# AnishDelft/ModelCompression

Measured on AMD Instinct MI355X. Metric: images/sec (fwd+bwd, 416x416), higher is better.
Workload: dtype fp16

## Files before the change

### modelcompression_amd/csrc/api.hip

```cpp
#include <stdarg.h>
#include <stdlib.h>
#include <string.h>

#include <string>

#include "kernels.h"

static thread_local char g_err[512] = "";

void mcamd_set_error(const char* fmt, ...) {
    va_list ap;
    va_start(ap, fmt);
    vsnprintf(g_err, sizeof(g_err), fmt, ap);
    va_end(ap);
}

int g_mcamd_env_generation = 0;
int McamdEnvSlot::get(const char* name, int dflt) {
    const int g = __atomic_load_n(&g_mcamd_env_generation, __ATOMIC_ACQUIRE);
    if (gen != g) {
        const char* s = getenv(name);
        has = s && *s ? 1 : 0;
        val = has ? atoi(s) : 0;
        __atomic_store_n(&gen, g, __ATOMIC_RELEASE);
// ... 1091 lines not shown
    if (!g || g->stem) return 0;
    const ConvRoute r = dgrad_route(g, concurrent != 0, MCAMD_EPI_RAW_F16);
    return mcamd_igemm_sums_ok(r) ? r.rows : 0;
}

extern "C" int mcamd_conv_dgrad_sums(const mcamd_conv_geom* g, const void* dy, int32_t dy_ld, int32_t dy_choff,
                                     const void* wp_dgrad, const mcamd_conv_epilogue* epi, const mcamd_dgrad_sums* sums,
                                     void* stream) {
    if (mcamd_recording()) {
        MCAMD_REQUIRE(g && epi, "conv_dgrad: null geometry / epilogue");
        const mcamd_conv_geom g_ = *g;
        const mcamd_conv_epilogue e_ = *epi;
        if (!sums) return mcamd_rec_push(stream, [=](void* s) { return mcamd_conv_dgrad_sums(&g_, dy, dy_ld, dy_choff, wp_dgrad, &e_, nullptr, s); });
        const mcamd_dgrad_sums s_ = *sums;
        return mcamd_rec_push(stream, [=](void* s) { return mcamd_conv_dgrad_sums(&g_, dy, dy_ld, dy_choff, wp_dgrad, &e_, &s_, s); });
    }
    if (check_geom(g, "conv_dgrad")) return MCAMD_EINVAL;
    MCAMD_REQUIRE(g->x_wrap == 0 && g->x_f8 == 0, "conv_dgrad: x_wrap / x_f8 are forward-only fields");
    MCAMD_REQUIRE(!g->stem, "conv_dgrad: the stem layer has no input gradient");
    MCAMD_REQUIRE(dy && wp_dgrad, "conv_dgrad: null input");
    int cout_p = cout_p_of(g);
    MCAMD_REQUIRE(dy_ld % 8 == 0 && dy_choff % 8 == 0 && dy_choff + cout_p <= dy_ld,
                  "conv_dgrad: dy slice [%d, %d) does not fit dy_ld %d", dy_choff, dy_choff + cout_p, dy_ld);
    IgemmArgs a;
    fill_operand(a, g, dy, wp_dgrad, dy_ld, dy_choff, g->cin, cout_p, 0);
    MCAMD_REQUIRE(epi && epi->mode != MCAMD_EPI_PAD_F16 && !epi->stats && epi->dst_mode == 0 && !epi->y2,
                  "conv_dgrad: epilogue must be mode 0 (no stats) or 1");
    a.concurrent = epi->concurrent != 0;
    const ConvRoute r = dgrad_route(g, a.concurrent, epi->mode);
    if (fill_epilogue(a, epi, g->cin, "conv_dgrad", r.rows)) return MCAMD_EINVAL;
    if (sums && sums->slab) {
        const mcamd_dgrad_sums* s = sums;
        MCAMD_REQUIRE(epi->mode == MCAMD_EPI_RAW_F16, "conv_dgrad: producer sums go with epilogue mode 0");
        MCAMD_REQUIRE(mcamd_igemm_sums_ok(r) && s->rows == r.rows,
                      "conv_dgrad: sums.rows must be mcamd_conv_dgrad_sums_rows() = %d (got %d; 0: this launch cannot take sums)",
                      mcamd_igemm_sums_ok(r) ? r.rows : 0, s->rows);
        MCAMD_REQUIRE(s->act && s->scale && s->shift && s->mean && s->invstd, "conv_dgrad: sums: null argument");
        MCAMD_REQUIRE(s->C > 0 && s->C % 8 == 0 && s->ch_lo >= 0 && s->ch_lo % 8 == 0 && s->ch_lo + s->C <= g->cin,
                      "conv_dgrad: sums: producer columns [%d, %d) must be whole groups of 8 inside the %d channels of G",
                      s->ch_lo, s->ch_lo + s->C, g->cin);
        MCAMD_REQUIRE(s->ld >= s->C, "conv_dgrad: sums.ld (%d) must be >= C (%d)", s->ld, s->C);
        MCAMD_REQUIRE(s->act_ld % 8 == 0 && s->act_choff % 8 == 0 && s->act_choff >= 0 && s->act_choff + s->C <= s->act_ld &&
                          (s->act_pad == 0 || s->act_pad == 1),
                      "conv_dgrad: sums: activation slice [%d, %d) does not fit act_ld %d", s->act_choff, s->act_choff + s->C, s->act_ld);
        MCAMD_REQUIRE(!s->y || (s->y_ld % 4 == 0 && s->y_choff % 4 == 0 && s->y_choff >= 0 && s->y_choff + s->C <= s->y_ld),
                      "conv_dgrad: sums: fp32 y slice [%d, %d) does not fit y_ld %d", s->y_choff, s->y_choff + s->C, s->y_ld);
        MCAMD_REQUIRE(s->slope > 0.f, "conv_dgrad: sums need an invertible activation (slope > 0)");
        a.bsum.slab = s->slab, a.bsum.ld = s->ld;
        a.bsum.act = (const half_t*)s->act, a.bsum.act_ld = s->act_ld, a.bsum.act_choff = s->act_choff, a.bsum.act_pw = s->act_pad ? 1 : 2;
        a.bsum.scale = s->scale, a.bsum.shift = s->shift, a.bsum.mean = s->mean, a.bsum.invstd = s->invstd;
        a.bsum.y = s->y, a.bsum.y_ld = s->y_ld, a.bsum.y_choff = s->y_choff;
        a.bsum.ch_lo = s->ch_lo, a.bsum.C = s->C;
        a.bsum.slope = s->slope;
    }
    return launch_route(a, r, g, (hipStream_t)stream);
}

extern "C" int mcamd_conv_dgrad(const mcamd_conv_geom* g, const void* dy, int32_t dy_ld, int32_t dy_choff,
                                const void* wp_dgrad, const mcamd_conv_epilogue* epi, void* stream) {
    return mcamd_conv_dgrad_sums(g, dy, dy_ld, dy_choff, wp_dgrad, epi, nullptr, stream);
}

static WgradPlan wgrad_plan_for(const mcamd_conv_geom* g) {
    if (mcamd_wgrad_stem_ok(g->stem, g->cout, g->W, (long long)g->B * g->H * g->W))
        return mcamd_wgrad_stem_plan((long long)g->B * g->H * g->W);
    if (mcamd_wgrad_win_ok(g->ksize, g->stem, g->cout, cin_tap_of(g), g->W, (long long)g->B * g->H * g->W))
        return mcamd_wgrad_win_plan((long long)g->B * g->H * g->W, g->cout);
    if (mcamd_wgrad_use9(g->ksize, g->stem, g->cout, cin_tap_of(g), g->W))
        return mcamd_wgrad_plan9(padded_pixels(g), g->cout, cin_tap_of(g), g->W, g->W + pw_of(g), g->B);
    return mcamd_wgrad_plan((long long)g->B * g->H * g->W, g->cout, cin_tap_of(g), ntaps_of(g));
}

extern "C" size_t mcamd_conv_wgrad_workspace_bytes(const mcamd_conv_geom* g) {
    if (!g) return 0;
    return wgrad_plan_for(g).bytes;
}

extern "C" int mcamd_conv_wgrad_plan_info(const mcamd_conv_geom* g, int32_t has_cmap, int32_t out[MCAMD_WGRAD_PLAN_INFO_N]) {
    if (check_geom(g, "conv_wgrad_plan_info")) return MCAMD_EINVAL;
    MCAMD_REQUIRE(out, "conv_wgrad_plan_info: null output");
    MCAMD_REQUIRE(!(g->stem && has_cmap), "conv_wgrad_plan_info: the stem layer takes no input-channel map");
    const WgradPlan p = wgrad_plan_for(g);
    const WgradFinish f = mcamd_wgrad_finish_pick(p.nsplit, g->stem, g->cin, g->ksize, has_cmap != 0);
    const int tiles = p.n_otiles * p.n_tapgroups * p.n_ctiles;
    out[0] = p.nine == 2 ? MCAMD_WGRAD_NINE_WIDE : p.nine ? MCAMD_WGRAD_NINE : p.stemw == 1 ? MCAMD_WGRAD_STEM
             : p.stemw == 2 ? MCAMD_WGRAD_WIN : MCAMD_WGRAD_GENERIC;
    out[1] = p.tmo, out[2] = p.tnc, out[3] = p.taps, out[4] = p.kp, out[5] = p.ns;
    out[6] = p.nsplit, out[7] = p.pix_per_split, out[8] = p.rows_pad;
    out[9] = f.kernel, out[10] = f.sg;
    out[11] = tiles;
    out[12] = p.stemw ? p.nsplit : round_up_int(tiles * p.nsplit, 8);
    return MCAMD_OK;
}

extern "C" int32_t mcamd_wgrad_generic_instances(int32_t* out, int32_t cap) {
    static_assert(sizeof(int32_t) == sizeof(int), "instance tuples are copied as int");
    return mcamd_wgrad_instances((int (*)[4])out, out ? cap : 0);
}

extern "C" int mcamd_conv_wgrad(const mcamd_conv_geom* g, const void* x, const void* dy, int32_t dy_ld, int32_t dy_choff,
                                const float* mask_oihw, const mcamd_chan_map* map, float grad_scale, float* dw_oihw,
                                float* dbias, void* workspace, size_t workspace_bytes, void* stream) {
    if (mcamd_recording()) {
        MCAMD_REQUIRE(g, "conv_wgrad: null geometry");
        const mcamd_conv_geom g_ = *g;
        const bool has_map = map != nullptr;
// ... 59 lines not shown
```

### modelcompression_amd/csrc/conv_epi.h

```cpp
#pragma once
#include "kernels.h"

__device__ __forceinline__ void split_image(int p, int HW, int& b, int& hw) {
    b = p / HW;
    hw = p - b * HW;
}
__device__ __forceinline__ void split_pixel(int p, int HW, int W, int& b, int& h, int& w) {
    int r;
    split_image(p, HW, b, r);
    h = r / W;
    w = r - h * W;
}

__device__ __forceinline__ void tile_pixel(const IgemmArgs& __restrict__ a, bool pooled, int m, int& b, int& h, int& w) {
    if (pooled) {
        const int Wo = a.W >> 1, q = m & 3;
        int ho, wo;
        split_pixel(m >> 2, (a.H >> 1) * Wo, Wo, b, ho, wo);
        h = 2 * ho + (q >> 1);
        w = 2 * wo + (q & 1);
    } else {
        split_pixel(m, a.HW, a.W, b, h, w);
    }
}

__device__ __forceinline__ long long tile_x_base(const IgemmArgs& __restrict__ a, bool pooled, int m) {
    if (m > a.M - 1) m = a.M - 1;
    int b, h, w;
    tile_pixel(a, pooled, m, b, h, w);
    return (long long)b * a.x_img_stride + (long long)h * a.x_row_stride + (long long)w * a.x_ld + a.x_off;
}

__device__ __forceinline__ bool xcd_tile(int num_ntiles, int num_slots, int& nt, int& slot) {
    const int xcd = blockIdx.x & 7, jb = blockIdx.x >> 3;
    nt = jb % num_ntiles;
    slot = (jb / num_ntiles) * 8 + xcd;
    return slot < num_slots;
}

__device__ __forceinline__ int e4m3_bytes4(const float* v) {
    float c[4];
#pragma unroll
    for (int e = 0; e < 4; ++e) c[e] = fminf(fmaxf(v[e] * 2.f, -448.f), 448.f);
    int w = __builtin_amdgcn_cvt_pk_fp8_f32(c[0], c[1], 0, false);
    return __builtin_amdgcn_cvt_pk_fp8_f32(c[2], c[3], w, true);
}

__device__ __forceinline__ h8_t q8_to_f16(int lo, int hi) {
    const h2_t p0 = __builtin_amdgcn_cvt_scalef32_pk_f16_fp8(lo, 1.0f, false), p1 = __builtin_amdgcn_cvt_scalef32_pk_f16_fp8(lo, 1.0f, true);
    const h2_t p2 = __builtin_amdgcn_cvt_scalef32_pk_f16_fp8(hi, 1.0f, false), p3 = __builtin_amdgcn_cvt_scalef32_pk_f16_fp8(hi, 1.0f, true);
    const h4_t a = __builtin_shufflevector(p0, p1, 0, 1, 2, 3), b = __builtin_shufflevector(p2, p3, 0, 1, 2, 3);
    return __builtin_shufflevector(a, b, 0, 1, 2, 3, 4, 5, 6, 7);
}

// ... 128 lines not shown
                                                 int pslot, int nt, int wm, int wn, int lane, int tid) {
    constexpr int TN = WN / 32;
#pragma unroll
    for (int j = 0; j < TN; ++j) {
        s1[j] += __shfl_xor(s1[j], 32);
        s2[j] += __shfl_xor(s2[j], 32);
    }
    __syncthreads();
    float* red = (float*)smem;
    if (lane < 32) {
#pragma unroll
        for (int j = 0; j < TN; ++j) {
            red[(wm * 2 + 0) * BN + wn * WN + j * 32 + lane] = s1[j];
            red[(wm * 2 + 1) * BN + wn * WN + j * 32 + lane] = s2[j];
        }
    }
    __syncthreads();
    for (int t = tid; t < 2 * BN; t += NT) {
        int which = t / BN, col = t - which * BN;
        float v = 0.f;
#pragma unroll
        for (int k = 0; k < BM / WM; ++k) v += red[(k * 2 + which) * BN + col];
        a.stats[((long long)pslot * 2 + which) * a.stats_ld + nt * BN + col] = v;
    }
}

__device__ __forceinline__ float bn_leaky(float y, float sc, float sh, float slope) {
    const float z = y * sc + sh;
    return z > 0.f ? z : z * slope;
}
__device__ __forceinline__ half_t sat_half(float v) {
    return (half_t)fminf(fmaxf(v, -65504.f), 65504.f);
}
__device__ __forceinline__ void split_hi_lo(const float* v, h8_t& hi, h8_t& lo) {
#pragma unroll
    for (int i = 0; i < 8; ++i) hi[i] = sat_half(v[i]);
#pragma unroll
    for (int i = 0; i < 8; ++i) lo[i] = (half_t)(v[i] - (float)hi[i]);
}

template <class T>
__device__ __forceinline__ const T* pin_here(const T* p) {
    asm volatile("" : "+s"(p));
    return p;
}
__host__ __device__ constexpr int sums_vals(int cols, int nt) { return (2 * cols + nt - 1) / nt; }
__host__ __device__ constexpr size_t sums_lds_bytes(int nt) { return (size_t)16 * (nt + 8) * sizeof(float); }

__host__ __device__ constexpr int sums_slots(int rows, int cols, int nt) { return rows * (cols / 8) / nt; }
__host__ __device__ constexpr int sums_early(int rows, int cols, int nt) {
    return rows * cols >= 256 * 256 && sums_slots(rows, cols, nt) > 8 ? 8 : sums_slots(rows, cols, nt);
}

template <int ROWS, int COLS, int NT>
__device__ __forceinline__ void sums_prefetch(const IgemmArgs& __restrict__ a, int mt, int nt, int tid,
                                              h8_t (&aq)[sums_early(ROWS, COLS, NT)]) {
    constexpr int CH = COLS / 8, RSTEP = NT / CH, NSLOT = sums_early(ROWS, COLS, NT);
    static_assert(NT % CH == 0 && (ROWS * CH) % NT == 0, "a thread keeps its 8 channels for all its slots");
    const int ch = tid % CH, row0 = tid / CH;
    const int n0 = nt * COLS + ch * 8;
    const int c = n0 - a.bsum.ch_lo;
    const bool live = n0 < a.N && c >= 0 && c < a.bsum.C;
    const half_t* act = pin_here(a.bsum.act) + a.bsum.act_choff + c;
    int m = mt * ROWS + row0;
    int b, h, w;
    split_pixel(m, a.HW, a.W, b, h, w);
    const int sb_ = RSTEP / a.HW, srem = RSTEP - sb_ * a.HW;
    const int sh_ = srem / a.W, sw_ = srem - sh_ * a.W;
#pragma unroll
    for (int k = 0; k < NSLOT; ++k) {
#pragma unroll
        for (int i = 0; i < 8; ++i) aq[k][i] = (half_t)0.f;
        if (live && m < a.M) aq[k] = *(const h8_t*)(act + pad_off(b, h, w, a.H, a.W, a.bsum.act_ld, a.bsum.act_pw));
        m += RSTEP;
        w += sw_;
        if (w >= a.W) w -= a.W, ++h;
        h += sh_;
        if (h >= a.H) h -= a.H, ++b;
        b += sb_;
    }
}

template <int ROWS, int COLS, int NT>
__device__ __forceinline__ void store_raw_tile_sums(const IgemmArgs& __restrict__ a, char* smem, int mt, int nt, int tid,
                                                    const h8_t (&aq)[sums_early(ROWS, COLS, NT)],
                                                    float (&tot)[sums_vals(COLS, NT)]) {
    constexpr int CH = COLS / 8, RSTEP = NT / CH, NSLOT = sums_slots(ROWS, COLS, NT), PITCH = NT + 8;
    constexpr int EARLY = sums_early(ROWS, COLS, NT);
    const half_t* ct = (const half_t*)smem;
    half_t* y = (half_t*)a.y;
    const int ch = tid % CH, row0 = tid / CH;
    const int n0 = nt * COLS + ch * 8;
    const int c = n0 - a.bsum.ch_lo;
    const bool col_ok = n0 < a.N;
    const bool live = col_ok && c >= 0 && c < a.bsum.C;
    float sb[8], sg[8], off[8], mul[8];
    bool usey[8];
    bool need_y = false;
#pragma unroll
    for (int i = 0; i < 8; ++i) sb[i] = sg[i] = 0.f, off[i] = 0.f, mul[i] = 0.f, usey[i] = false;
    if (live) {
        const float *scp = pin_here(a.bsum.scale) + c, *shp = pin_here(a.bsum.shift) + c;
        const float *mup = pin_here(a.bsum.mean) + c, *isp = pin_here(a.bsum.invstd) + c;
        float sc[8], sh[8], mu[8], is[8];
#pragma unroll
        for (int i = 0; i < 8; ++i) sc[i] = scp[i], sh[i] = shp[i], mu[i] = mup[i], is[i] = isp[i];
        need_y = act_xhat_source(sc, sh, mu, is, a.bsum.y != nullptr, off, mul, usey);
    }
    const float slope = a.bsum.slope, inv_slope = 1.0f / slope;
#pragma unroll
    for (int k = 0; k < NSLOT; ++k) {
        const int row = row0 + k * RSTEP, m = mt * ROWS + row;
        if (!col_ok || m >= a.M) continue;
        const h8_t gq = *(const h8_t*)(ct + row * COLS + ch * 8);
        *(h8_t*)(y + (long long)m * a.y_ld + a.y_choff + n0) = gq;
        if (!live) continue;
        h8_t av8;
        if (k < EARLY) {
            av8 = aq[k];
        } else {
            int b, h, w;
            split_pixel(m, a.HW, a.W, b, h, w);
            av8 = *(const h8_t*)(a.bsum.act + pad_off(b, h, w, a.H, a.W, a.bsum.act_ld, a.bsum.act_pw) + a.bsum.act_choff + c);
        }
        float z[8];
#pragma unroll
        for (int i = 0; i < 8; ++i) {
            const float av = (float)av8[i];
            z[i] = av > 0.f ? av : av * inv_slope;
        }
        if (need_y) {
            const float* yp = a.bsum.y + (long long)m * a.bsum.y_ld + a.bsum.y_choff + c;
#pragma unroll
            for (int i = 0; i < 8; ++i) z[i] = usey[i] ? yp[i] : z[i];
        }
#pragma unroll
        for (int i = 0; i < 8; ++i) {
            const float gv = (float)gq[i];
            const float gz = (float)av8[i] > 0.f ? gv : gv * slope;
            sb[i] += gz;
            sg[i] += gz * ((z[i] - off[i]) * mul[i]);
        }
    }
    __syncthreads();
    float* red = (float*)smem;
#pragma unroll
    for (int i = 0; i < 8; ++i) {
        red[i * PITCH + tid] = sb[i];
        red[(8 + i) * PITCH + tid] = sg[i];
    }
    __syncthreads();
#pragma unroll
    for (int k = 0; k < sums_vals(COLS, NT); ++k) {
        const int t = tid + k * NT;
        if (t < 2 * COLS) {
            const int which = t / COLS, col = t - which * COLS;
            const int v = which * 8 + (col & 7), chq = col >> 3;
            float s = 0.f;
            for (int r = 0; r < RSTEP; ++r) s += red[v * PITCH + r * CH + chq];
            tot[k] += s;
        }
    }
}

template <int COLS, int NT>
__device__ __forceinline__ void store_tile_sums_slab(const IgemmArgs& __restrict__ a, int pslot, int nt, int tid,
                                                     const float (&tot)[sums_vals(COLS, NT)]) {
#pragma unroll
    for (int k = 0; k < sums_vals(COLS, NT); ++k) {
        const int t = tid + k * NT;
        if (t < 2 * COLS) {
            const int which = t / COLS, col = t - which * COLS;
            const int n = nt * COLS + col, c = n - a.bsum.ch_lo;
            if (n < a.N && c >= 0 && c < a.bsum.C) a.bsum.slab[((long long)pslot * 2 + which) * a.bsum.ld + c] = tot[k];
        }
    }
}

struct NoBorder {
    static constexpr bool on = false;
};
struct Q8Border {
    static constexpr bool on = true;
    const float* table;
    const int* wexp;
    int ld, m0;
    __device__ __forceinline__ int cls(const IgemmArgs& __restrict__ a, int pix) const {
        int m = m0 + pix, b, h, w;
        if (m > a.M - 1) m = a.M - 1;
        tile_pixel(a, a.dst_mode != 0, m, b, h, w);
        return (h == 0 ? 1 : 0) | (h == a.H - 1 ? 2 : 0) | (w == 0 ? 4 : 0) | (w == a.W - 1 ? 8 : 0);
    }
    __device__ __forceinline__ float pre(int n) const { return ldexpf(1.f, -(wexp[n] + 1)); }
    __device__ __forceinline__ f32x4_t row(int c, int n0) const { return *(const f32x4_t*)(table + c * ld + n0); }
};

// ... 126 lines not shown
```

### modelcompression_amd/csrc/conv_igemm.hip

```cpp
#include "kernels.h"
#include "conv_epi.h"
#include <stdlib.h>


template <int BM, int BN, int WM, int WN, int BK, int NSTAGE, int EPI>
__global__ __launch_bounds__((BM / WM) * (BN / WN) * 64,
                              (BN >= 128 ? (NSTAGE * BK <= 96 ? 3 : 2) : (BN >= 64 ? 3 : 4)))
void igemm_kernel(IgemmArgs a) {
    constexpr int WAVES_N = BN / WN;
    constexpr int NT = (BM / WM) * (BN / WN) * 64;
    constexpr int CPR = BK / 8;
    constexpr int A_SLOTS = BM * CPR, B_SLOTS = BN * CPR;
    constexpr int A_IT = (A_SLOTS + NT - 1) / NT, B_IT = (B_SLOTS + NT - 1) / NT;
    constexpr int TM = WM / 32, TN = WN / 32;
    constexpr int STAGE_BYTES = (A_SLOTS + B_SLOTS) * 16;
    constexpr int DMIN = A_SLOTS / NT + B_SLOTS / NT;
    static_assert(A_SLOTS % 64 == 0 && B_SLOTS % 64 == 0, "whole waves per DMA instruction");
    static_assert(NSTAGE >= 2 && NSTAGE <= 4 && DMIN * (NSTAGE - 2) < 64, "vmcnt immediate range");

    extern __shared__ __attribute__((aligned(16))) char smem[];

    const int tid = threadIdx.x;
    const int lane = tid & 63;
    const int wave = __builtin_amdgcn_readfirstlane(tid >> 6);
    const int wm = wave / WAVES_N, wn = wave % WAVES_N;
    int nt, pslot;
    if (a.xcd_order == 0) {
        const int total_items = a.num_ntiles * a.num_pslots;
        const int chunk = (total_items + 7) >> 3;
        const int item = (blockIdx.x & 7) * chunk + (blockIdx.x >> 3);
        if ((int)(blockIdx.x >> 3) >= chunk || item >= total_items) return;
        nt = item / a.num_pslots;
        pslot = item - nt * a.num_pslots;
    } else {
        if (!xcd_tile(a.num_ntiles, a.num_pslots, nt, pslot)) return;
    }
    const int nchunks = a.ktot / BK;
    const int cpt = a.cin_tap / BK;

    long long bbase[B_IT];
#pragma unroll
    for (int it = 0; it < B_IT; ++it) {
        int slot = it * NT + tid;
        int row = slot / CPR, phys = slot % CPR;
        int logical = phys ^ swz<CPR>(row);
        bbase[it] = (long long)(nt * BN + row) * a.ktot + logical * 8;
    }

    float s1[TN], s2[TN];
#pragma unroll
    for (int j = 0; j < TN; ++j) s1[j] = s2[j] = 0.f;
    bool sat = false;
    constexpr bool SUMS = EPI == MCAMD_EPI_RAW_F16_SUMS;
    float tot[SUMS ? sums_vals(BN, NT) : 1];
#pragma unroll
    for (int k = 0; k < (SUMS ? sums_vals(BN, NT) : 1); ++k) tot[k] = 0.f;

    for (int mt = pslot; mt < a.num_mtiles; mt += a.num_pslots) {
        long long abase[A_IT];
#pragma unroll
        for (int it = 0; it < A_IT; ++it) {
            int slot = it * NT + tid;
            int row = slot / CPR, phys = slot % CPR;
            int logical = phys ^ swz<CPR>(row);
            abase[it] = tile_x_base(a, EPI == MCAMD_EPI_PAD_F16 && a.dst_mode != 0, mt * BM + row) + logical * 8;
        }

        f32x16_t acc[TM][TN];
#pragma unroll
        for (int i = 0; i < TM; ++i)
#pragma unroll
            for (int j = 0; j < TN; ++j)
#pragma unroll
                for (int r = 0; r < 16; ++r) acc[i][j][r] = 0.f;

        auto stage = [&](int q, int buf) {
            const int sub = a.kb / BK > 0 ? a.kb / BK : 1, per_block = a.ntaps * sub;
            const int cb = q / per_block, r = q - cb * per_block;
            const int tap = r / sub;
            int cbo = cb * a.kb;
            if (cbo >= a.wrap) cbo -= a.wrap;
            int koff = a.tap_off[tap] + cbo + (r - tap * sub) * BK;
            char* sa = smem + buf * STAGE_BYTES;
            char* sb = sa + A_SLOTS * 16;
#pragma unroll
            for (int it = 0; it < A_IT; ++it) {
                int wslot = it * NT + wave * 64;
                if (wslot < A_SLOTS) glds16(a.x + abase[it] + koff, sa + wslot * 16);
            }
#pragma unroll
            for (int it = 0; it < B_IT; ++it) {
                int wslot = it * NT + wave * 64;
                if (wslot < B_SLOTS) glds16(a.w + bbase[it] + (long long)q * BK, sb + wslot * 16);
            }
        };

        __syncthreads();
#pragma unroll
        for (int p = 0; p < NSTAGE - 1; ++p)
            if (p < nchunks) stage(p, p);
        int sidx = 0;
        for (int q = 0; q < nchunks; ++q) {
            int issued = q + NSTAGE - 1;
            if (issued > nchunks) issued = nchunks;
            const int inflight = issued - q - 1;
            if (NSTAGE == 2 || inflight == 0) wait_vmcnt<0>();
            else if (inflight == 1) wait_vmcnt<DMIN>();
            else wait_vmcnt<(NSTAGE > 3 ? 2 * DMIN : DMIN)>();
            __builtin_amdgcn_s_barrier();
            if (q + NSTAGE - 1 < nchunks) {
                int ns = sidx + NSTAGE - 1;
                if (ns >= NSTAGE) ns -= NSTAGE;
                stage(q + NSTAGE - 1, ns);
            }
            const char* sa = smem + sidx * STAGE_BYTES;
            const char* sb = sa + A_SLOTS * 16;
            sidx = sidx + 1 == NSTAGE ? 0 : sidx + 1;
            constexpr int KS = BK / 16;
            constexpr int NSET = (TM * TN <= 4) ? 2 : 1;
            h8_t af[NSET][TM], bf[NSET][TN];
            auto load_frags = [&](int s, int set) {
                const int chunk = 2 * s + (lane >> 5);
#pragma unroll
                for (int i = 0; i < TM; ++i) {
                    int row = wm * WM + i * 32 + (lane & 31);
                    af[set][i] = *(const h8_t*)(sa + (row * CPR + (chunk ^ swz<CPR>(row))) * 16);
                }
#pragma unroll
                for (int j = 0; j < TN; ++j) {
                    int row = wn * WN + j * 32 + (lane & 31);
                    bf[set][j] = *(const h8_t*)(sb + (row * CPR + (chunk ^ swz<CPR>(row))) * 16);
                }
            };
            if (NSET == 2) load_frags(0, 0);
#pragma unroll
            for (int s = 0; s < KS; ++s) {
                if (NSET == 2) {
                    if (s + 1 < KS) load_frags(s + 1, (s + 1) & 1);
                    __builtin_amdgcn_sched_barrier(0);
                } else {
                    load_frags(s, 0);
                }
                constexpr int M1 = NSET - 1;
#pragma unroll
                for (int i = 0; i < TM; ++i)
#pragma unroll
                    for (int j = 0; j < TN; ++j)
                        acc[i][j] = __builtin_amdgcn_mfma_f32_32x32x16_f16(af[s & M1][i], bf[s & M1][j], acc[i][j], 0, 0, 0);
                if (NSET == 2) __builtin_amdgcn_sched_barrier(0);
            }
        }

        if constexpr (EPI == MCAMD_EPI_NCHW_F32) {
            float* y = (float*)a.y;
#pragma unroll
            for (int i = 0; i < TM; ++i)
#pragma unroll
                for (int r = 0; r < 16; ++r) {
                    int m = mt * BM + wm * WM + i * 32 + mfma32_row(r, lane);
                    if (m < a.M) {
                        int b, hw;
                        split_image(m, a.HW, b, hw);
#pragma unroll
                        for (int j = 0; j < TN; ++j) {
                            int n = nt * BN + wn * WN + j * 32 + (lane & 31);
                            if (n < a.N) {
                                float v = acc[i][j][r];
                                if (a.bias) v += a.bias[n];
                                y[((long long)b * a.N + n) * a.HW + hw] = v;
                            }
                        }
                    }
                }
        } else if constexpr (EPI == MCAMD_EPI_RAW_F32) {
            store_raw32_tile<BM, BN, WM, WN>(a, acc, mt, nt, wm, wn, lane, s1, s2);
        } else {
            h8_t aq[SUMS ? sums_early(BM, BN, NT) : 1];
            if constexpr (SUMS) sums_prefetch<BM, BN, NT>(a, mt, nt, tid, aq);
            __syncthreads();
            half_t* ct = (half_t*)smem;
            const int mlim = a.M - mt * BM;
#pragma unroll
            for (int j = 0; j < TN; ++j) {
                const int col = wn * WN + j * 32 + (lane & 31);
                float sc = 1.f, sh = 0.f;
                if constexpr (EPI == MCAMD_EPI_PAD_F16) {
                    int n = nt * BN + col;
                    if (n < a.N) {
                        if (a.scale) sc = a.scale[n];
                        if (a.shift) sh = a.shift[n];
                    }
                }
#pragma unroll
                for (int i = 0; i < TM; ++i)
#pragma unroll
                    for (int r = 0; r < 16; ++r) {
                        const int row = wm * WM + i * 32 + mfma32_row(r, lane);
                        float v = acc[i][j][r];
                        if constexpr (EPI == MCAMD_EPI_PAD_F16) {
                            v = v * sc + sh;
                            v = v > 0.f ? v : v * a.slope;
                        }
                        half_t hv = (half_t)fminf(fmaxf(v, -65504.f), 65504.f);
                        sat |= fabsf(v) > 65504.f;
                        ct[row * BN + col] = hv;
                        if (EPI == MCAMD_EPI_RAW_F16 && a.stats) {
                            float fv = (row < mlim) ? (float)hv : 0.f;
                            s1[j] += fv;
                            s2[j] += fv * fv;
                        }
                    }
            }
            __syncthreads();
            if constexpr (EPI == MCAMD_EPI_PAD_F16) store_pad_tile<BM, BN, BN, NT>(a, nullptr, ct, false, false, mt, nt, tid);
            else if constexpr (SUMS) store_raw_tile_sums<BM, BN, NT>(a, smem, mt, nt, tid, aq, tot);
            else store_raw_tile<BM, BN, NT>(a, ct, mt, nt, tid);
        }
    }

    if (sat && a.overflow) atomicOr(a.overflow, 1);
    if constexpr (SUMS) store_tile_sums_slab<BN, NT>(a, pslot, nt, tid, tot);
    if ((EPI == MCAMD_EPI_RAW_F16 || EPI == MCAMD_EPI_RAW_F32) && a.stats)
        store_stats_slab<BM, BN, WM, WN, NT>(a, smem, s1, s2, pslot, nt, wm, wn, lane, tid);
}

struct TileCfg {
    int bm, bn, bk;
    int kind;
};

static TileCfg pick_tile(long long M, int n, int cin_tap, int ktot, bool raw_epilogue = true, bool concurrent = false) {
    TileCfg t;
    t.kind = 0;
    if (raw_epilogue && mcamd_small3x3_ok(M, n, cin_tap, ktot)) {
        t.bm = 32, t.bn = round_up_int(n, 32), t.bk = cin_tap, t.kind = 4;
        return t;
    }
    {
        const int pp = MCAMD_ENV_INT("MCAMD_PP", 1);
        if (pp && ktot >= 256 && n >= 128 && M >= 256) {
            bool use = pp == 2;
            int bm = 256, bn = 256;
            if (pp == 1 && ktot >= 1152) {
                double best_cost = -1.0, best_span = 0.0;
                const int bms[2] = {256, 192}, bns[2] = {256, 128};
                for (int cn = 0; cn < 2; ++cn) {
                    if (n < bns[cn]) continue;
                    for (int c = 0; c < 2; ++c) {
                        const long long tiles = ((M + bms[c] - 1) / bms[c]) * ((n + bns[cn] - 1) / bns[cn]);
                        const long long rounds = (tiles + 255) / 256;
                        const double fill = (double)tiles / (double)(rounds * 256);
                        const double rate = bns[cn] == 256 ? 1.0 : 0.8;
                        if (fill < 0.8 && !(concurrent && rounds == 1 && fill >= 0.4)) continue;
                        const double span = (double)rounds * bms[c] * bns[cn] / rate;
                        const double cost = concurrent ? (double)tiles * bms[c] * bns[cn] / rate : span;
                        const bool better = best_cost < 0 || (concurrent ? (cost < 0.97 * best_cost || (cost < 1.03 * best_cost && span < best_span))
                                                                         : cost < best_cost);
                        if (better) best_cost = cost, best_span = span, bm = bms[c], bn = bns[cn];
                    }
                }
                use = best_cost >= 0;
            }
            if (pp >= 2) {
                if (MCAMD_ENV_INT("MCAMD_PP_BM", 256) == 192) bm = 192;
                if (MCAMD_ENV_INT("MCAMD_PP_BN", 256) == 128) bn = 128;
            }
            if (use) {
                t.bm = bm, t.bn = bn, t.bk = 32, t.kind = 2;
// ... 99 lines not shown
```

### modelcompression_amd/csrc/conv_igemm_pp.hip

```cpp
#include "kernels.h"
#include "conv_epi.h"
#include <stdlib.h>

namespace {

constexpr int BK = 32, NST = 4;
constexpr int WAVES_N = 4;
constexpr int NT = 512;
constexpr int CPR = BK / 8;

template <int MS> struct Shape;
template <> struct Shape<32> {
    typedef f32x16_t acc_t;
    static constexpr int AR = 16, KS = 2;
    __device__ static __forceinline__ int swz4(int row) { return (row >> 2) & 3; }
    __device__ static __forceinline__ int rowof(int r, int lane) { return mfma32_row(r, lane); }
    __device__ static __forceinline__ acc_t mfma(h8_t a, h8_t b, acc_t c) {
        return __builtin_amdgcn_mfma_f32_32x32x16_f16(a, b, c, 0, 0, 0);
    }
};
template <> struct Shape<16> {
    typedef f32x4_t acc_t;
    static constexpr int AR = 4, KS = 1;
    __device__ static __forceinline__ int swz4(int row) {
// ... 18 lines not shown
}

template <int EPI, int BM, int BN, int MS, bool F8 = false>
__global__ __launch_bounds__(512, 1) void igemm_pp_kernel(IgemmArgs a) {
    static_assert(!F8 || MS == 32, "the fp8 correction chunks are 32x32x64 blocks");
    typedef Shape<MS> SH;
    typedef typename SH::acc_t acc_v;
    constexpr int AR = SH::AR, KS = SH::KS;
    constexpr int WN = BN / WAVES_N, B_SLOTS = BN * CPR, B_IT = B_SLOTS / NT;
    static_assert(BN == 256 || BN == 128, "wave tiles of 64 or 32 columns");
    constexpr int WM = BM / 2, TM = WM / MS, TN = WN / MS;
    constexpr int A_SLOTS = BM * CPR;
    constexpr int A_IT = (A_SLOTS + NT - 1) / NT;
    constexpr bool RAGGED = A_SLOTS % NT != 0;
    constexpr int DPC = A_IT + B_IT;
    constexpr int STAGE_BYTES = (A_SLOTS + B_SLOTS) * 16;
    static_assert(BM == 256 || BM == 192, "wave tiles of 128 or 96 rows");
    extern __shared__ __attribute__((aligned(16))) char smem[];
    const int tid = threadIdx.x, lane = tid & 63;
    const int wave = __builtin_amdgcn_readfirstlane(tid >> 6);
    const int wm = wave / WAVES_N, wn = wave % WAVES_N;
    const int group = wave >> 2;
    auto wait_chunks = [&](int n) {
        if (RAGGED && group == 1) {
            if (n == 2) wait_vmcnt<2 * (DPC - 1)>();
            else if (n == 1) wait_vmcnt<DPC - 1>();
            else wait_vmcnt<0>();
        } else {
            if (n == 2) wait_vmcnt<2 * DPC>();
            else if (n == 1) wait_vmcnt<DPC>();
            else wait_vmcnt<0>();
        }
    };

    int nt, pslot;
    if (!xcd_tile(a.num_ntiles, a.num_pslots, nt, pslot)) return;
    const int nchunks = a.ktot / BK;
    const int cpt = a.cin_tap / BK;

    long long bbase[B_IT];
#pragma unroll
    for (int it = 0; it < B_IT; ++it) {
        const int slot = it * NT + tid;
        const int row = slot / CPR, phys = slot % CPR;
        bbase[it] = (long long)(nt * BN + row) * a.ktot + (phys ^ SH::swz4(row)) * 8;
    }

    float s1[TN], s2[TN];
#pragma unroll
    for (int j = 0; j < TN; ++j) s1[j] = s2[j] = 0.f;
    bool sat = false;
    constexpr bool SUMS = EPI == MCAMD_EPI_RAW_F16_SUMS;
    float tot[SUMS ? sums_vals(BN, NT) : 1];
#pragma unroll
    for (int k = 0; k < (SUMS ? sums_vals(BN, NT) : 1); ++k) tot[k] = 0.f;

    for (int mt = pslot; mt < a.num_mtiles; mt += a.num_pslots) {
        long long abase[A_IT];
#pragma unroll
        for (int it = 0; it < A_IT; ++it) {
            const int slot = it * NT + tid;
            const int row = (slot / CPR) % BM, phys = slot % CPR;
            abase[it] = tile_x_base(a, EPI == MCAMD_EPI_PAD_F16 && a.dst_mode != 0, mt * BM + row) + (phys ^ SH::swz4(row)) * 8;
        }

        acc_v acc[TM][TN];
#pragma unroll
        for (int i = 0; i < TM; ++i)
#pragma unroll
            for (int j = 0; j < TN; ++j)
#pragma unroll
                for (int r = 0; r < AR; ++r) acc[i][j][r] = 0.f;

        const char* aptr[A_IT];
        const char* bptr[B_IT];
#pragma unroll
        for (int it = 0; it < A_IT; ++it) aptr[it] = (const char*)(a.x + abase[it]);
#pragma unroll
        for (int it = 0; it < B_IT; ++it) bptr[it] = (const char*)(a.w + bbase[it]);
        int st_cb = 0, st_tap = 0, st_c = 0, st_q = 0;
        auto stage_next = [&]() {
            const int koff = (a.tap_off[st_tap] + (st_cb >= a.wrap ? st_cb - a.wrap : st_cb) + st_c) * 2;
            const int woff = st_q * (BK * 2);
            char* sa = smem + (st_q & (NST - 1)) * STAGE_BYTES;
            char* sb = sa + A_SLOTS * 16;
#pragma unroll
            for (int it = 0; it < A_IT; ++it)
                if (it * NT + wave * 64 < A_SLOTS) glds16(aptr[it] + koff, sa + (it * NT + wave * 64) * 16);
#pragma unroll
            for (int it = 0; it < B_IT; ++it) glds16(bptr[it] + woff, sb + (it * NT + wave * 64) * 16);
            ++st_q;
            st_c += BK;
            if (st_c == a.kb) {
                st_c = 0;
                if (++st_tap == a.ntaps) {
                    st_tap = 0;
                    st_cb += a.kb;
                }
            }
        };
        const int lrow = lane & (MS - 1);
        const int c0 = (lane / MS) ^ SH::swz4(lrow);
        const int a_off0 = ((wm * WM + lrow) * CPR + c0) * 16, a_off1 = ((wm * WM + lrow) * CPR + (c0 ^ 2)) * 16;
        const int b_off0 = A_SLOTS * 16 + ((wn * WN + lrow) * CPR + c0) * 16;
        const int b_off1 = A_SLOTS * 16 + ((wn * WN + lrow) * CPR + (c0 ^ 2)) * 16;

        __syncthreads();
#pragma unroll
        for (int q = 0; q < NST - 1; ++q)
            if (q < nchunks) stage_next();
        wait_chunks(nchunks >= 3 ? 2 : nchunks - 1);
        __builtin_amdgcn_s_barrier();
        if (group == 1) __builtin_amdgcn_s_barrier();

        auto chunk_phases = [&](const int p, const bool IS8) __attribute__((always_inline)) {
            __builtin_amdgcn_sched_barrier(0);
            const bool more = p + NST - 1 < nchunks;
            const int koff = (a.tap_off[st_tap] + (st_cb >= a.wrap ? st_cb - a.wrap : st_cb) + st_c) * 2;
            const int woff = st_q * (BK * 2);
            char* sa = smem + (st_q & (NST - 1)) * STAGE_BYTES;
            char* sb = sa + A_SLOTS * 16;
            auto issue_piece = [&](int piece) {
                if (piece < A_IT) {
                    if (piece * NT + wave * 64 < A_SLOTS) glds16(aptr[piece] + koff, sa + (piece * NT + wave * 64) * 16);
                } else if (piece - A_IT < B_IT) {
                    glds16(bptr[piece - A_IT] + woff, sb + ((piece - A_IT) * NT + wave * 64) * 16);
                }
            };
            wait_chunks(p + 2 < nchunks ? 1 : 0);
            const char* sbase = smem + (p & (NST - 1)) * STAGE_BYTES;
            h8_t af[F8 ? 1 : KS][F8 ? 1 : TM], bf[F8 ? 1 : KS][F8 ? 1 : TN];
            i32x8_t af8[F8 ? TM : 1], bf8[F8 ? TN : 1];
            if constexpr (F8) {
#pragma unroll
                for (int j = 0; j < TN; ++j) bf8[j] = read_pair(sbase + b_off0 + j * (MS * CPR * 16), sbase + b_off1 + j * (MS * CPR * 16));
#pragma unroll
                for (int i = 0; i < TM; ++i) af8[i] = read_pair(sbase + a_off0 + i * (MS * CPR * 16), sbase + a_off1 + i * (MS * CPR * 16));
            } else {
#pragma unroll
                for (int j = 0; j < TN; ++j) {
                    bf[0][j] = *(const h8_t*)(sbase + b_off0 + j * (MS * CPR * 16));
                    if (KS == 2) bf[KS - 1][j] = *(const h8_t*)(sbase + b_off1 + j * (MS * CPR * 16));
                }
#pragma unroll
                for (int i = 0; i < TM; ++i) {
                    af[0][i] = *(const h8_t*)(sbase + a_off0 + i * (MS * CPR * 16));
                    if (KS == 2) af[KS - 1][i] = *(const h8_t*)(sbase + a_off1 + i * (MS * CPR * 16));
                }
            }
            asm volatile("s_waitcnt lgkmcnt(0)" ::: "memory");
            __builtin_amdgcn_sched_barrier(0);
            __builtin_amdgcn_s_barrier();
            __builtin_amdgcn_sched_barrier(0);
            __builtin_amdgcn_s_setprio(1);
            bool did8 = false;
            if constexpr (F8) {
                if (IS8) {
                    did8 = true;
                    const int SA = 127 * 0x01010101, SB = a.f8_sb;
#pragma unroll
// ... 42 lines not shown
            __builtin_amdgcn_s_barrier();
        };
        {
            const int p8 = F8 ? (a.f8_from < nchunks ? a.f8_from : nchunks) : nchunks;
            int p = 0;
            for (; p < p8; ++p) chunk_phases(p, false);
            if constexpr (F8)
                for (; p < nchunks; ++p) chunk_phases(p, true);
        }
        if (group == 0) __builtin_amdgcn_s_barrier();
        if constexpr (F8) asm volatile("s_nop 15\n\ts_nop 15" ::: "memory");

        if constexpr (EPI == MCAMD_EPI_NCHW_F32) {
            float* y = (float*)a.y;
#pragma unroll
            for (int i = 0; i < TM; ++i)
#pragma unroll
                for (int r = 0; r < AR; ++r) {
                    const int m = mt * BM + wm * WM + i * MS + SH::rowof(r, lane);
                    if (m < a.M) {
                        int b, hw;
                        split_image(m, a.HW, b, hw);
#pragma unroll
                        for (int j = 0; j < TN; ++j) {
                            const int n = nt * BN + wn * WN + j * MS + (lane & (MS - 1));
                            if (n < a.N) {
                                float v = acc[i][j][r];
                                if (a.bias) v += a.bias[n];
                                y[((long long)b * a.N + n) * a.HW + hw] = v;
                            }
                        }
                    }
                }
        } else if constexpr (EPI == MCAMD_EPI_RAW_F32) {
            float* y = (float*)a.y;
            const int mlim = a.M - mt * BM;
#pragma unroll
            for (int j = 0; j < TN; ++j) {
                const int n = nt * BN + wn * WN + j * MS + (lane & (MS - 1));
#pragma unroll
                for (int i = 0; i < TM; ++i)
#pragma unroll
                    for (int r = 0; r < AR; ++r) {
                        const int row = wm * WM + i * MS + SH::rowof(r, lane);
                        const float v = acc[i][j][r];
                        if (row < mlim) {
                            if (n < a.N) y[(long long)(mt * BM + row) * a.y_ld + a.y_choff + n] = v;
                            s1[j] += v;
                            s2[j] += v * v;
                        }
                    }
            }
        } else {
            h8_t aq[SUMS ? sums_early(BM, BN, NT) : 1];
            if constexpr (SUMS) sums_prefetch<BM, BN, NT>(a, mt, nt, tid, aq);
            __syncthreads();
            half_t* ct = (half_t*)smem;
            const int mlim = a.M - mt * BM;
#pragma unroll
            for (int j = 0; j < TN; ++j) {
                const int col = wn * WN + j * MS + (lane & (MS - 1));
                float sc = 1.f, sh = 0.f;
                if constexpr (EPI == MCAMD_EPI_PAD_F16) {
                    const int n = nt * BN + col;
                    if (n < a.N) {
                        if (a.scale) sc = a.scale[n];
                        if (a.shift) sh = a.shift[n];
                    }
                }
#pragma unroll
                for (int i = 0; i < TM; ++i)
#pragma unroll
                    for (int r = 0; r < AR; ++r) {
                        const int row = wm * WM + i * MS + SH::rowof(r, lane);
                        float v = acc[i][j][r];
                        if constexpr (EPI == MCAMD_EPI_PAD_F16) {
                            v = v * sc + sh;
                            v = v > 0.f ? v : v * a.slope;
                        }
                        const half_t hv = (half_t)fminf(fmaxf(v, -65504.f), 65504.f);
                        sat |= fabsf(v) > 65504.f;
                        ct[row * BN + col] = hv;
                        if (EPI == MCAMD_EPI_RAW_F16 && a.stats) {
                            const float fv = (row < mlim) ? (float)hv : 0.f;
                            s1[j] += fv;
                            s2[j] += fv * fv;
                        }
                    }
            }
            __syncthreads();
            if constexpr (EPI == MCAMD_EPI_PAD_F16) store_pad_tile<BM, BN, BN, NT>(a, nullptr, ct, false, false, mt, nt, tid);
            else if constexpr (SUMS) store_raw_tile_sums<BM, BN, NT>(a, smem, mt, nt, tid, aq, tot);
            else store_raw_tile<BM, BN, NT>(a, ct, mt, nt, tid);
        }
    }

    if (sat && a.overflow) atomicOr(a.overflow, 1);
    if constexpr (SUMS) store_tile_sums_slab<BN, NT>(a, pslot, nt, tid, tot);
    if ((EPI == MCAMD_EPI_RAW_F16 || EPI == MCAMD_EPI_RAW_F32) && a.stats) {
#pragma unroll
        for (int j = 0; j < TN; ++j) {
            s1[j] += __shfl_xor(s1[j], 32);
            s2[j] += __shfl_xor(s2[j], 32);
            if (MS == 16) {
                s1[j] += __shfl_xor(s1[j], 16);
                s2[j] += __shfl_xor(s2[j], 16);
            }
        }
        __syncthreads();
        float* red = (float*)smem;
        if (lane < MS) {
#pragma unroll
            for (int j = 0; j < TN; ++j) {
                red[(wm * 2 + 0) * BN + wn * WN + j * MS + lane] = s1[j];
                red[(wm * 2 + 1) * BN + wn * WN + j * MS + lane] = s2[j];
            }
        }
        __syncthreads();
        for (int t = tid; t < 2 * BN; t += NT) {
            const int which = t / BN, col = t - which * BN;
            float v = 0.f;
#pragma unroll
            for (int k = 0; k < BM / WM; ++k) v += red[(k * 2 + which) * BN + col];
            a.stats[((long long)pslot * 2 + which) * a.stats_ld + nt * BN + col] = v;
        }
    }
}

template <int EPI, int BM, int BN, int MS, bool F8 = false>
static void launch_pp(const IgemmArgs& a, int rows, int ntiles, hipStream_t st) {
    constexpr size_t ring = (size_t)NST * (BM + BN) * CPR * 16;
    static_assert((size_t)BM * BN * 2 <= ring && sums_lds_bytes(NT) <= ring, "output tile (and the partials of the sums form) fit the ring");
    MCAMD_LDS_OPT_IN((igemm_pp_kernel<EPI, BM, BN, MS, F8>), ring);
    hipLaunchKernelGGL((igemm_pp_kernel<EPI, BM, BN, MS, F8>), dim3(round_up_int(rows, 8) * ntiles + 8), dim3(NT), ring, st, a);
}

int mcamd_igemm_pp_launch(const IgemmArgs& a, int bm, int bn, int rows, int ntiles, hipStream_t st) {
    if (a.cin_tap % BK != 0 || a.ktot < BK || a.kb % BK != 0 || (bm != 256 && bm != 192) || (bn != 256 && bn != 128)) {
        mcamd_set_error("igemm_pp: K per tap (%d) must be a multiple of %d, tile (%d x %d) 256|192 x 256|128", a.cin_tap, BK, bm, bn);
        return MCAMD_EINVAL;
    }
    if (a.f8_from != 0x7fffffff) {
        if (a.mode != MCAMD_EPI_RAW_F32 || a.f8_from <= 0 || a.f8_from >= a.ktot / BK || a.wrap != 0x7fffffff) {
            mcamd_set_error("igemm_pp: the fp8 correction form needs epilogue mode 3, no x_wrap and 0 < f8_from (%d) < chunks", a.f8_from);
            return MCAMD_EINVAL;
// ... 32 lines not shown
```

### modelcompression_amd/csrc/kernels.h

```cpp
#pragma once
#include "common.h"

struct DgradSums {
    float* slab;
    const half_t* act;
    const float* scale;
    const float* shift;
    const float* mean;
    const float* invstd;
    const float* y;
    int act_ld, act_choff, act_pw;
    int y_ld, y_choff;
    int ch_lo, C;
    int ld;
    float slope;
};
#define MCAMD_EPI_RAW_F16_SUMS 4

struct IgemmArgs {
    const half_t* x;
    const half_t* w;
    void* y;
    const float* bias;
    float* stats;
    const float* scale;
    const float* shift;
    long long x_img_stride;
    int x_row_stride;
    int x_ld;
    int x_off;
    int H, W, HW, M, N;
    int ktot;
    int cin_tap;
    int ntaps;
    int kb;
    int tap_off[9];
    int mode;
    int y_ld, y_choff;
    int stats_ld;
    float slope;
    int num_mtiles;
    int num_pslots;
    int num_ntiles;
    int xcd_order;
    int* overflow;
    int dst_mode;
    void* y2;
    int y2_ld, y2_choff;
    int concurrent;
    int wrap;
    int f8_from;
    int f8_sb;
    DgradSums bsum;
};


struct StemArgs {
    const half_t* x;
    const half_t* w;
    half_t* y;
    float* stats;
    int y_ld, y_choff, stats_ld;
    int H, W, HW, M;
};

struct WgradArgs {
    const half_t* x;
    const half_t* dy;
// ... 123 lines not shown
```

Baseline: 5649.

## Prefetch dgrad sums activations before the K loop and specialize the no-y path

In the dgrad kernels with the fused BN-sums epilogue, the activation loads for the epilogue are issued before the main K loop for selected tile shapes, so their latency overlaps the GEMM instead of stalling the epilogue. The loads use global address-space pointers. The sums loop also gets a wave-uniform specialization that skips the fp32 y path when no lane needs it. An env flag (on by default) enables the early prefetch. The risk is extra registers held live across the main loop, which may lower occupancy.

```diff
diff --git a/modelcompression_amd/csrc/api.hip b/modelcompression_amd/csrc/api.hip
--- a/modelcompression_amd/csrc/api.hip
+++ b/modelcompression_amd/csrc/api.hip
@@ -1167,6 +1167,7 @@
         a.bsum.y = s->y, a.bsum.y_ld = s->y_ld, a.bsum.y_choff = s->y_choff;
         a.bsum.ch_lo = s->ch_lo, a.bsum.C = s->C;
         a.bsum.slope = s->slope;
+        a.bsum.early = MCAMD_ENV_INT("MCAMD_DGRAD_SUMS_EARLY", 1) != 0;
     }
     return launch_route(a, r, g, (hipStream_t)stream);
 }
diff --git a/modelcompression_amd/csrc/conv_epi.h b/modelcompression_amd/csrc/conv_epi.h
--- a/modelcompression_amd/csrc/conv_epi.h
+++ b/modelcompression_amd/csrc/conv_epi.h
@@ -1,5 +1,6 @@
 #pragma once
 #include "kernels.h"
+#include <type_traits>
 
 __device__ __forceinline__ void split_image(int p, int HW, int& b, int& hw) {
     b = p / HW;
@@ -234,44 +235,48 @@
     return rows * cols >= 256 * 256 && sums_slots(rows, cols, nt) > 8 ? 8 : sums_slots(rows, cols, nt);
 }
 
-template <int ROWS, int COLS, int NT>
+template <int ROWS, int COLS, int NT, int FIRST, int LAST>
 __device__ __forceinline__ void sums_prefetch(const IgemmArgs& __restrict__ a, int mt, int nt, int tid,
                                               h8_t (&aq)[sums_early(ROWS, COLS, NT)]) {
-    constexpr int CH = COLS / 8, RSTEP = NT / CH, NSLOT = sums_early(ROWS, COLS, NT);
+    constexpr int CH = COLS / 8, RSTEP = NT / CH;
     static_assert(NT % CH == 0 && (ROWS * CH) % NT == 0, "a thread keeps its 8 channels for all its slots");
-    const int ch = tid % CH, row0 = tid / CH;
-    const int n0 = nt * COLS + ch * 8;
-    const int c = n0 - a.bsum.ch_lo;
-    const bool live = n0 < a.N && c >= 0 && c < a.bsum.C;
-    const half_t* act = pin_here(a.bsum.act) + a.bsum.act_choff + c;
-    int m = mt * ROWS + row0;
-    int b, h, w;
-    split_pixel(m, a.HW, a.W, b, h, w);
-    const int sb_ = RSTEP / a.HW, srem = RSTEP - sb_ * a.HW;
-    const int sh_ = srem / a.W, sw_ = srem - sh_ * a.W;
-#pragma unroll
-    for (int k = 0; k < NSLOT; ++k) {
-#pragma unroll
-        for (int i = 0; i < 8; ++i) aq[k][i] = (half_t)0.f;
-        if (live && m < a.M) aq[k] = *(const h8_t*)(act + pad_off(b, h, w, a.H, a.W, a.bsum.act_ld, a.bsum.act_pw));
-        m += RSTEP;
-        w += sw_;
-        if (w >= a.W) w -= a.W, ++h;
-        h += sh_;
-        if (h >= a.H) h -= a.H, ++b;
-        b += sb_;
-    }
-}
-
-template <int ROWS, int COLS, int NT>
+    static_assert(FIRST >= 0 && FIRST <= LAST && LAST <= sums_early(ROWS, COLS, NT), "pieces of aq[]");
+    if constexpr (FIRST < LAST) {
+        typedef const __attribute__((address_space(1))) h8_t* gptr_t;
+        const int ch = tid % CH, row0 = tid / CH;
+        const int n0 = nt * COLS + ch * 8;
+        const int c = n0 - a.bsum.ch_lo;
+        const bool live = n0 < a.N && c >= 0 && c < a.bsum.C;
+        const half_t* act = pin_here(a.bsum.act) + a.bsum.act_choff + c;
+        int m = mt * ROWS + row0 + FIRST * RSTEP;
+        int b, h, w;
+        split_pixel(m, a.HW, a.W, b, h, w);
+        const int sb_ = RSTEP / a.HW, srem = RSTEP - sb_ * a.HW;
+        const int sh_ = srem / a.W, sw_ = srem - sh_ * a.W;
+#pragma unroll
+        for (int k = FIRST; k < LAST; ++k) {
+#pragma unroll
+            for (int i = 0; i < 8; ++i) aq[k][i] = (half_t)0.f;
+            if (live && m < a.M) aq[k] = *(gptr_t)(act + pad_off(b, h, w, a.H, a.W, a.bsum.act_ld, a.bsum.act_pw));
+            m += RSTEP;
+            w += sw_;
+            if (w >= a.W) w -= a.W, ++h;
+            h += sh_;
+            if (h >= a.H) h -= a.H, ++b;
+            b += sb_;
+        }
+    }
+}
+
+template <int ROWS, int COLS, int NT, bool SPLIT>
 __device__ __forceinline__ void store_raw_tile_sums(const IgemmArgs& __restrict__ a, char* smem, int mt, int nt, int tid,
                                                     const h8_t (&aq)[sums_early(ROWS, COLS, NT)],
                                                     float (&tot)[sums_vals(COLS, NT)]) {
     constexpr int CH = COLS / 8, RSTEP = NT / CH, NSLOT = sums_slots(ROWS, COLS, NT), PITCH = NT + 8;
     constexpr int EARLY = sums_early(ROWS, COLS, NT);
-    const half_t* ct = (const half_t*)smem;
     half_t* y = (half_t*)a.y;
     const int ch = tid % CH, row0 = tid / CH;
+    const half_t* ct0 = (const half_t*)smem + row0 * COLS + ch * 8;
     const int n0 = nt * COLS + ch * 8;
     const int c = n0 - a.bsum.ch_lo;
     const bool col_ok = n0 < a.N;
@@ -290,40 +295,46 @@
         need_y = act_xhat_source(sc, sh, mu, is, a.bsum.y != nullptr, off, mul, usey);
     }
     const float slope = a.bsum.slope, inv_slope = 1.0f / slope;
-#pragma unroll
-    for (int k = 0; k < NSLOT; ++k) {
-        const int row = row0 + k * RSTEP, m = mt * ROWS + row;
-        if (!col_ok || m >= a.M) continue;
-        const h8_t gq = *(const h8_t*)(ct + row * COLS + ch * 8);
-        *(h8_t*)(y + (long long)m * a.y_ld + a.y_choff + n0) = gq;
-        if (!live) continue;
-        h8_t av8;
-        if (k < EARLY) {
-            av8 = aq[k];
-        } else {
-            int b, h, w;
-            split_pixel(m, a.HW, a.W, b, h, w);
-            av8 = *(const h8_t*)(a.bsum.act + pad_off(b, h, w, a.H, a.W, a.bsum.act_ld, a.bsum.act_pw) + a.bsum.act_choff + c);
-        }
-        float z[8];
-#pragma unroll
-        for (int i = 0; i < 8; ++i) {
-            const float av = (float)av8[i];
-            z[i] = av > 0.f ? av : av * inv_slope;
-        }
-        if (need_y) {
-            const float* yp = a.bsum.y + (long long)m * a.bsum.y_ld + a.bsum.y_choff + c;
-#pragma unroll
-            for (int i = 0; i < 8; ++i) z[i] = usey[i] ? yp[i] : z[i];
-        }
-#pragma unroll
-        for (int i = 0; i < 8; ++i) {
-            const float gv = (float)gq[i];
-            const float gz = (float)av8[i] > 0.f ? gv : gv * slope;
-            sb[i] += gz;
-            sg[i] += gz * ((z[i] - off[i]) * mul[i]);
-        }
-    }
+    auto slots = [&](auto with_y) __attribute__((always_inline)) {
+#pragma unroll
+        for (int k = 0; k < NSLOT; ++k) {
+            const int row = row0 + k * RSTEP, m = mt * ROWS + row;
+            if (!col_ok || m >= a.M) continue;
+            const h8_t gq = *(const h8_t*)(ct0 + k * RSTEP * COLS);
+            *(h8_t*)(y + (long long)m * a.y_ld + a.y_choff + n0) = gq;
+            if (!live) continue;
+            h8_t av8;
+            if (k < EARLY) {
+                av8 = aq[k < EARLY ? k : 0];
+            } else {
+                int b, h, w;
+                split_pixel(m, a.HW, a.W, b, h, w);
+                av8 = *(const h8_t*)(a.bsum.act + pad_off(b, h, w, a.H, a.W, a.bsum.act_ld, a.bsum.act_pw) + a.bsum.act_choff + c);
+            }
+            float z[8];
+#pragma unroll
+            for (int i = 0; i < 8; ++i) {
+                const float av = (float)av8[i];
+                z[i] = av > 0.f ? av : av * inv_slope;
+            }
+            if constexpr (decltype(with_y)::value) {
+                if (need_y) {
+                    const float* yp = a.bsum.y + (long long)m * a.bsum.y_ld + a.bsum.y_choff + c;
+#pragma unroll
+                    for (int i = 0; i < 8; ++i) z[i] = usey[i] ? yp[i] : z[i];
+                }
+            }
+#pragma unroll
+            for (int i = 0; i < 8; ++i) {
+                const float gv = (float)gq[i];
+                const float gz = (float)av8[i] > 0.f ? gv : gv * slope;
+                sb[i] += gz;
+                sg[i] += gz * ((z[i] - off[i]) * mul[i]);
+            }
+        }
+    };
+    if (!SPLIT || __builtin_amdgcn_ballot_w64(need_y) != 0) slots(std::true_type());
+    else slots(std::false_type());
     __syncthreads();
     float* red = (float*)smem;
 #pragma unroll
diff --git a/modelcompression_amd/csrc/conv_igemm.hip b/modelcompression_amd/csrc/conv_igemm.hip
--- a/modelcompression_amd/csrc/conv_igemm.hip
+++ b/modelcompression_amd/csrc/conv_igemm.hip
@@ -53,6 +53,7 @@
     bool sat = false;
     constexpr bool SUMS = EPI == MCAMD_EPI_RAW_F16_SUMS;
     float tot[SUMS ? sums_vals(BN, NT) : 1];
+    constexpr int SUMS_K = SUMS && BM == 128 && (BN == 64 || NSTAGE == 2) ? sums_early(BM, BN, NT) : 0;
 #pragma unroll
     for (int k = 0; k < (SUMS ? sums_vals(BN, NT) : 1); ++k) tot[k] = 0.f;
 
@@ -96,6 +97,12 @@
         };
 
         __syncthreads();
+        h8_t aq[SUMS ? sums_early(BM, BN, NT) : 1];
+        const bool sums_under_k = SUMS_K > 0 && a.bsum.early;
+        if constexpr (SUMS_K > 0) {
+            if (sums_under_k) sums_prefetch<BM, BN, NT, 0, SUMS_K>(a, mt, nt, tid, aq);
+            __builtin_amdgcn_sched_barrier(0);
+        }
 #pragma unroll
         for (int p = 0; p < NSTAGE - 1; ++p)
             if (p < nchunks) stage(p, p);
@@ -175,8 +182,10 @@
         } else if constexpr (EPI == MCAMD_EPI_RAW_F32) {
             store_raw32_tile<BM, BN, WM, WN>(a, acc, mt, nt, wm, wn, lane, s1, s2);
         } else {
-            h8_t aq[SUMS ? sums_early(BM, BN, NT) : 1];
-            if constexpr (SUMS) sums_prefetch<BM, BN, NT>(a, mt, nt, tid, aq);
+            if constexpr (SUMS) {
+                if (!sums_under_k) sums_prefetch<BM, BN, NT, 0, SUMS_K>(a, mt, nt, tid, aq);
+                sums_prefetch<BM, BN, NT, SUMS_K, sums_early(BM, BN, NT)>(a, mt, nt, tid, aq);
+            }
             __syncthreads();
             half_t* ct = (half_t*)smem;
             const int mlim = a.M - mt * BM;
@@ -213,7 +222,7 @@
             }
             __syncthreads();
             if constexpr (EPI == MCAMD_EPI_PAD_F16) store_pad_tile<BM, BN, BN, NT>(a, nullptr, ct, false, false, mt, nt, tid);
-            else if constexpr (SUMS) store_raw_tile_sums<BM, BN, NT>(a, smem, mt, nt, tid, aq, tot);
+            else if constexpr (SUMS) store_raw_tile_sums<BM, BN, NT, BM == 128>(a, smem, mt, nt, tid, aq, tot);
             else store_raw_tile<BM, BN, NT>(a, ct, mt, nt, tid);
         }
     }
diff --git a/modelcompression_amd/csrc/conv_igemm_pp.hip b/modelcompression_amd/csrc/conv_igemm_pp.hip
--- a/modelcompression_amd/csrc/conv_igemm_pp.hip
+++ b/modelcompression_amd/csrc/conv_igemm_pp.hip
@@ -94,6 +94,8 @@
     bool sat = false;
     constexpr bool SUMS = EPI == MCAMD_EPI_RAW_F16_SUMS;
     float tot[SUMS ? sums_vals(BN, NT) : 1];
+    constexpr int SUMS_K = SUMS && BM * BN == 192 * 128 ? sums_early(BM, BN, NT) : 0;
+    constexpr bool SUMS_SPLIT = BM * BN < 256 * 256;
 #pragma unroll
     for (int k = 0; k < (SUMS ? sums_vals(BN, NT) : 1); ++k) tot[k] = 0.f;
 
@@ -148,6 +150,12 @@
         const int b_off1 = A_SLOTS * 16 + ((wn * WN + lrow) * CPR + (c0 ^ 2)) * 16;
 
         __syncthreads();
+        h8_t aq[SUMS ? sums_early(BM, BN, NT) : 1];
+        const bool sums_under_k = SUMS_K > 0 && a.bsum.early;
+        if constexpr (SUMS_K > 0) {
+            if (sums_under_k) sums_prefetch<BM, BN, NT, 0, SUMS_K>(a, mt, nt, tid, aq);
+            __builtin_amdgcn_sched_barrier(0);
+        }
 #pragma unroll
         for (int q = 0; q < NST - 1; ++q)
             if (q < nchunks) stage_next();
@@ -296,8 +304,10 @@
                     }
             }
         } else {
-            h8_t aq[SUMS ? sums_early(BM, BN, NT) : 1];
-            if constexpr (SUMS) sums_prefetch<BM, BN, NT>(a, mt, nt, tid, aq);
+            if constexpr (SUMS) {
+                if (!sums_under_k) sums_prefetch<BM, BN, NT, 0, SUMS_K>(a, mt, nt, tid, aq);
+                sums_prefetch<BM, BN, NT, SUMS_K, sums_early(BM, BN, NT)>(a, mt, nt, tid, aq);
+            }
             __syncthreads();
             half_t* ct = (half_t*)smem;
             const int mlim = a.M - mt * BM;
@@ -334,7 +344,7 @@
             }
             __syncthreads();
             if constexpr (EPI == MCAMD_EPI_PAD_F16) store_pad_tile<BM, BN, BN, NT>(a, nullptr, ct, false, false, mt, nt, tid);
-            else if constexpr (SUMS) store_raw_tile_sums<BM, BN, NT>(a, smem, mt, nt, tid, aq, tot);
+            else if constexpr (SUMS) store_raw_tile_sums<BM, BN, NT, SUMS_SPLIT>(a, smem, mt, nt, tid, aq, tot);
             else store_raw_tile<BM, BN, NT>(a, ct, mt, nt, tid);
         }
     }
diff --git a/modelcompression_amd/csrc/kernels.h b/modelcompression_amd/csrc/kernels.h
--- a/modelcompression_amd/csrc/kernels.h
+++ b/modelcompression_amd/csrc/kernels.h
@@ -14,6 +14,7 @@
     int ch_lo, C;
     int ld;
     float slope;
+    int early;
 };
 #define MCAMD_EPI_RAW_F16_SUMS 4
 
```

After: 5659 (median of 6 runs). Within noise of the previous version (+0.2%).
